# djene-mengistu/UAPS

Measured on AMD Instinct MI355X. Metric: training images/sec (labeled+unlabeled) NEU-Seg 256x256 K=3, higher is better.
Workload: dtype f32

## Files before the change

include/uaps_hip.h:

```cpp
#ifndef UAPS_HIP_H
#define UAPS_HIP_H

#include <stddef.h>
#include <stdint.h>

#ifdef __cplusplus
extern "C" {
#endif

typedef void* uaps_stream_t;

#define UAPS_MAX_HEADS 8
#define UAPS_MAX_CLASSES 8

#define UAPS_OK 0
#define UAPS_EINVAL (-1)
#define UAPS_ERANGE (-2)
#define UAPS_EWORKSPACE (-3)
#define UAPS_ENOFORM (-4)

int uaps_abi_version(void);
const char* uaps_error_string(int code);


// ... 426 lines not shown
#define UAPS_BIN_S_KBCE 15
#define UAPS_BIN_S_KFOCAL 16
#define UAPS_BIN_S_NSCALARS 24
int uaps_binloss_workspace_bytes(int B, int H, int W, size_t* out_host);
int uaps_binloss_fwd(const float* z, const void* target, const uaps_binloss_params* prm, int B, int H, int W, float* scalars,
                     void* workspace, size_t workspace_bytes, uaps_stream_t stream);
int uaps_binloss_bwd(const float* z, const void* target, const uaps_binloss_params* prm, const float* scalars, const float* grad,
                     int B, int H, int W, float* dz, uaps_stream_t stream);
int uaps_sigmoid_mse_fwd(const float* a, const float* b, long n, float* out, uaps_stream_t stream);
int uaps_sigmoid_mse_bwd(const float* a, const float* b, const float* g_map, long n, float* da, uaps_stream_t stream);
int uaps_sigmoid_kl_fwd(const float* a, const float* b, long n, float* out_mean, void* workspace, size_t workspace_bytes,
                        uaps_stream_t stream);
int uaps_sigmoid_kl_bwd(const float* a, const float* b, const float* grad, long n, float* da, uaps_stream_t stream);
int uaps_bin_confusion(const float* z, const int64_t* labels, int B, int H, int W, double threshold, int64_t* counts,
                       uaps_stream_t stream);

int uaps_add_relu(const float* a, const float* b, float* out, long n, uaps_stream_t stream);
int uaps_relu_bwd(const float* dout, const float* out, float* dx, long n, uaps_stream_t stream);
int uaps_bn_act_bwd_prepare(const float* dout, const float* y, const float* gamma, const float* beta, const float* save_mean,
                            const float* save_invstd, float slope, int B, int C, int H, int W, int groups, float* coef,
                            float* dgamma, float* dbeta, float* dconv_bias, float* dy_bound, void* workspace, size_t workspace_bytes,
                            uaps_stream_t stream);
int uaps_bn_act_bwd_finalize(const void* partials, int parts_per_image, const float* maxes, const float* gamma, const float* beta,
                             const float* save_mean, const float* save_invstd, int B, int C, int H, int W, int groups, float* coef,
                             float* dgamma, float* dbeta, float* dconv_bias, float* dy_bound, uaps_stream_t stream);
int uaps_bn_act_bwd_apply(const float* dout, const float* y, const float* coef, float slope, int B, int C, int H, int W, int groups,
                          float* dy, uaps_stream_t stream);
int uaps_head_bwd_fused(const float* dlogits, const float* y, const void* xf, float slope, int groups, const float* wb,
                        const float* dy_bound, float dy_mul, const float* x_bound, float x_mul, const float* save_mean,
                        const float* save_invstd, const float* gamma, const float* beta, int want_bias, int B, int Cin, int Cout,
                        int H, int W, int ks, int cfg, float* g, void* partials, float* maxes, void* workspace,
                        size_t workspace_bytes, uaps_stream_t stream);

int uaps_relu_bwd_sum(const float* const* dout_host, int k, const float* out, float* dx, long n, uaps_stream_t stream);

int uaps_cat2(const float* a, const float* b, float* out, long n, uaps_stream_t stream);

int uaps_augment_batch(const uint8_t* images_hwc, const uint8_t* masks, const int* params_i, const float* params_f,
                       const float* noise, uint64_t seed, int B, int Hs, int Ws, int Ho, int Wo, const float* mean3_host,
                       const float* std3_host, float* out, int64_t* out_mask, uaps_stream_t stream);

#define UAPS_AUG_END 0
#define UAPS_AUG_BC 1
#define UAPS_AUG_NOISE 2
#define UAPS_AUG_BLUR 3
#define UAPS_AUG_BRIGHT 4
#define UAPS_AUG_CONTRAST 5
#define UAPS_AUG_SATURATE 6
#define UAPS_AUG_HUE 7
#define UAPS_AUG_PIXDROP 8
#define UAPS_AUG_GRID 9
#define UAPS_AUG_MAX_OPS 8
typedef struct uaps_view_row {
    int32_t hflip, vflip, rot_k, grid_on;
    int32_t op[UAPS_AUG_MAX_OPS];
    float a[UAPS_AUG_MAX_OPS], b[UAPS_AUG_MAX_OPS];
} uaps_view_row;
typedef struct uaps_augment_views_call {
    uint32_t struct_size;
    int32_t V, B, Hs, Ws, Cs, Ho, Wo;
    const uint8_t* images;
    const uint8_t* masks;
    const uaps_view_row* rows_host;
    const uaps_view_row* rows;
    const float* grid_ys;
    const float* grid_xs;
// ... 281 lines not shown
```

uaps_amd/_lib.py:

```python
from __future__ import annotations

import ctypes as C
import os
import subprocess
import threading

from . import config

_HERE = os.path.dirname(os.path.abspath(__file__))
LIB_PATH = config.text("UAPS_HIP_LIB") or os.path.join(_HERE, "lib", "libuaps_hip.so")
CSRC = os.path.join(_HERE, "csrc")

_lock = threading.Lock()
_tls = threading.local()
_lib = None

c_float_p = C.POINTER(C.c_float)
c_void_p = C.c_void_p

_PTR = C.c_void_p
SIGNATURES = {
    "uaps_abi_version": (C.c_int, []),
    "uaps_error_string": (C.c_char_p, [C.c_int]),
    "uaps_loss_workspace_bytes": (C.c_int, [C.c_int] * 5 + [C.POINTER(C.c_size_t)]),
# ... 65 lines not shown
    "uaps_convs_fwd": (C.c_int, [_PTR] * 3 + [C.c_int] * 8 + [_PTR]),
    "uaps_convs_bwd_data": (C.c_int, [_PTR] * 3 + [C.c_int] * 8 + [_PTR]),
    "uaps_convs_wrw_workspace_bytes": (C.c_int, [C.c_int] * 8 + [C.POINTER(C.c_size_t)]),
    "uaps_convs_bwd_weight": (C.c_int, [_PTR] * 3 + [C.c_int] * 8 + [_PTR, C.c_size_t, _PTR]),
    "uaps_maxpool3x3s2_fwd": (C.c_int, [_PTR, _PTR, _PTR, C.c_long, C.c_int, C.c_int, _PTR]),
    "uaps_maxpool3x3s2_bwd": (C.c_int, [_PTR, _PTR, _PTR, C.c_long, C.c_int, C.c_int, _PTR]),
    "uaps_space_to_depth2": (C.c_int, [_PTR, _PTR, C.c_int, C.c_int, C.c_int, C.c_int, C.c_int, _PTR]),
    "uaps_subsample2_fwd": (C.c_int, [_PTR, _PTR, C.c_long, C.c_int, C.c_int, _PTR]),
    "uaps_subsample2_bwd": (C.c_int, [_PTR, _PTR, C.c_long, C.c_int, C.c_int, _PTR]),
    "uaps_sum_tensors": (C.c_int, [_PTR, C.c_int, _PTR, C.c_long, _PTR]),
    "uaps_pair_workspace_bytes": (C.c_int, [C.POINTER(C.c_size_t)]),
    "uaps_feat_dropout_stats": (C.c_int, [_PTR] + [C.c_int] * 4 + [_PTR, C.c_size_t, _PTR]),
    "uaps_fanout_perturbed": (C.c_int, [_PTR] * 7 + [C.c_int, C.c_int, C.c_uint64, C.c_float, C.c_float] + [C.c_int] * 4 + [_PTR]),
    "uaps_augment_batch": (C.c_int, [_PTR] * 5 + [C.c_uint64] + [C.c_int] * 5 + [C.POINTER(C.c_float), C.POINTER(C.c_float), _PTR, _PTR, _PTR]),
    "uaps_augment_views_workspace_bytes": (C.c_int, [C.c_int] * 4 + [C.POINTER(C.c_size_t)]),
    "uaps_augment_views": (C.c_int, [_PTR]),
    "uaps_softmax_klmap_bwd": (C.c_int, [_PTR] * 3 + [C.c_int] * 4 + [_PTR] * 3),
    "uaps_softmax_pair_fwd": (C.c_int, [_PTR, _PTR] + [C.c_int] * 5 + [_PTR, _PTR, _PTR, _PTR, C.c_size_t, _PTR]),
    "uaps_softmax_mse_bwd": (C.c_int, [_PTR] * 3 + [C.c_int] * 4 + [_PTR, _PTR]),
    "uaps_softmax_kl_bwd": (C.c_int, [_PTR] * 3 + [C.c_int] * 4 + [_PTR, _PTR]),
    "uaps_entropy_map": (C.c_int, [_PTR] + [C.c_int] * 4 + [_PTR, _PTR, _PTR, C.c_size_t, _PTR]),
    "uaps_fanin_perturbed": (C.c_int, [_PTR] * 4 + [C.c_int, C.c_int, C.c_uint64, C.c_float, C.c_float] + [C.c_int] * 4 + [_PTR, _PTR]),
    "uaps_maxpool2x2_fwd": (C.c_int, [_PTR] + [C.c_int] * 4 + [_PTR, _PTR, _PTR]),
    "uaps_adam_step": (C.c_int, [_PTR] * 5 + [C.c_int] + [C.c_double] * 5 + [C.c_long, _PTR]),
    "uaps_add_relu": (C.c_int, [_PTR, _PTR, _PTR, C.c_long, _PTR]),
    "uaps_relu_bwd": (C.c_int, [_PTR, _PTR, _PTR, C.c_long, _PTR]),
    "uaps_relu_bwd_sum": (C.c_int, [_PTR, C.c_int, _PTR, _PTR, C.c_long, _PTR]),
    "uaps_cat2": (C.c_int, [_PTR, _PTR, _PTR, C.c_long, _PTR]),
    "uaps_bn_act_bwd_prepare": (C.c_int, [_PTR] * 6 + [C.c_float] + [C.c_int] * 5 + [_PTR] * 6 + [C.c_size_t, _PTR]),
    "uaps_bn_act_bwd_apply": (C.c_int, [_PTR] * 3 + [C.c_float] + [C.c_int] * 5 + [_PTR, _PTR]),
    "uaps_bn_act_bwd_finalize": (C.c_int, [_PTR, C.c_int] + [_PTR] * 5 + [C.c_int] * 5 + [_PTR] * 6),
    "uaps_head_bwd_fused": (C.c_int, [_PTR] * 3 + [C.c_float, C.c_int, _PTR, _PTR, C.c_float, _PTR, C.c_float] + [_PTR] * 4 + [C.c_int] * 8 +
                            [_PTR] * 4 + [C.c_size_t, _PTR]),
    "uaps_seg_confusion": (C.c_int, [_PTR, _PTR] + [C.c_int] * 4 + [_PTR, _PTR]),
    "uaps_ema_update": (C.c_int, [_PTR] * 3 + [C.c_int, C.c_float, C.c_float, _PTR]),
    "uaps_teacher_noise": (C.c_int, [_PTR] + [C.c_int] * 5 + [C.c_uint64, C.c_uint64, _PTR, _PTR]),
    "uaps_teacher_noise_apply": (C.c_int, [_PTR, _PTR] + [C.c_int] * 5 + [_PTR, _PTR]),
    "uaps_mc_consistency_workspace_bytes": (C.c_int, [C.POINTER(C.c_size_t)]),
    "uaps_mc_consistency_fwd": (C.c_int, [_PTR] * 3 + [C.c_int] * 5 + [C.c_float] + [_PTR] * 4 + [C.c_size_t, _PTR]),
    "uaps_mc_consistency_bwd": (C.c_int, [_PTR] * 5 + [C.c_int] * 4 + [_PTR, _PTR]),
    "uaps_cct_dct_workspace_bytes": (C.c_int, [C.POINTER(C.c_size_t)]),
    "uaps_cct_consistency_fwd": (C.c_int, [_PTR] + [C.c_int] * 6 + [_PTR, _PTR, C.c_size_t, _PTR]),
    "uaps_cct_consistency_bwd": (C.c_int, [_PTR] + [C.c_int] * 6 + [_PTR, _PTR, _PTR]),
    "uaps_rot90_batch": (C.c_int, [_PTR, _PTR] + [C.c_int] * 5 + [_PTR, _PTR, _PTR]),
    "uaps_rot_consistency_fwd": (C.c_int, [_PTR, C.c_int, _PTR] + [C.c_int] * 6 + [_PTR, _PTR, C.c_size_t, _PTR]),
    "uaps_rot_consistency_bwd": (C.c_int, [_PTR, C.c_int, _PTR] + [C.c_int] * 6 + [_PTR, _PTR, _PTR, _PTR]),
    "uaps_cps_workspace_bytes": (C.c_int, [C.c_int] * 5 + [C.POINTER(C.c_size_t)]),
    "uaps_cps_fwd": (C.c_int, [_PTR] * 3 + [C.c_int] * 5 + [C.c_float] + [_PTR] * 4 + [C.c_size_t, _PTR]),
    "uaps_cps_bwd": (C.c_int, [_PTR] * 7 + [C.c_int] * 5 + [_PTR] * 3),
    "uaps_ucc_cutmix_batch": (C.c_int, [_PTR] * 6 + [C.c_int] * 4 + [_PTR] * 3),
    "uaps_ucc_workspace_bytes": (C.c_int, [C.c_int] * 4 + [C.POINTER(C.c_size_t)]),
    "uaps_ucc_fwd": (C.c_int, [_PTR] * 3 + [C.c_int] * 4 + [C.c_float] + [_PTR] * 6 + [C.c_size_t, _PTR]),
    "uaps_ucc_bwd": (C.c_int, [_PTR] * 6 + [C.c_int] * 4 + [_PTR] * 3),
    "uaps_segloss_workspace_bytes": (C.c_int, [C.c_int] * 4 + [C.POINTER(C.c_size_t)]),
    "uaps_segloss_fwd": (C.c_int, [_PTR] * 3 + [C.c_int] * 4 + [_PTR, _PTR, C.c_size_t, _PTR]),
    "uaps_segloss_bwd": (C.c_int, [_PTR] * 5 + [C.c_int] * 4 + [_PTR, _PTR]),
    "uaps_binloss_workspace_bytes": (C.c_int, [C.c_int] * 3 + [C.POINTER(C.c_size_t)]),
    "uaps_binloss_fwd": (C.c_int, [_PTR] * 3 + [C.c_int] * 3 + [_PTR, _PTR, C.c_size_t, _PTR]),
    "uaps_binloss_bwd": (C.c_int, [_PTR] * 5 + [C.c_int] * 3 + [_PTR, _PTR]),
    "uaps_sigmoid_mse_fwd": (C.c_int, [_PTR, _PTR, C.c_long, _PTR, _PTR]),
    "uaps_sigmoid_mse_bwd": (C.c_int, [_PTR, _PTR, _PTR, C.c_long, _PTR, _PTR]),
    "uaps_sigmoid_kl_fwd": (C.c_int, [_PTR, _PTR, C.c_long, _PTR, _PTR, C.c_size_t, _PTR]),
    "uaps_sigmoid_kl_bwd": (C.c_int, [_PTR, _PTR, _PTR, C.c_long, _PTR, _PTR]),
    "uaps_bin_confusion": (C.c_int, [_PTR, _PTR] + [C.c_int] * 3 + [C.c_double, _PTR, _PTR]),
    "uaps_tta_views": (C.c_int, [_PTR]),
    "uaps_tta_fold": (C.c_int, [_PTR]),
# ... 388 lines not shown
```

uaps_amd/config.py:

```python
from __future__ import annotations

import os
from typing import Dict

_seen: Dict[str, tuple] = {}

DOC = {
    "UAPS_HIP_LIB": "path of another build of libuaps_hip.so with the same ABI (same-box A/B of two kernel builds)",
    "UAPS_CONV_MODE": "arithmetic of the convolutions: 2 / h16 (default), 1 / split (exact three-piece bf16), 0 / exact (fp32 MFMA)",
    "UAPS_DEFER_WRW_REDUCE": "weight-gradient reductions batched behind the backward (conv.deferred_reduces)",
    "UAPS_EARLY_WRW_REDUCE": "... and the decoders' share of them on a side stream beside the encoder's backward",
    "UAPS_EARLY_ADAM": "the decoders' Adam step behind their early reductions (world size 1)",
    "UAPS_FUSED_UP2": "bilinear x2 formed in the staging of up4's first convolution instead of materialised",
    "UAPS_FUSED_BN_SUMS": "BatchNorm-backward sums in the epilogue of the 16 -> 16 input-gradient row kernel (measured a wash: off)",
    "UAPS_FUSED_HEAD_BWD": "out_conv's input gradient, weight gradient and the BatchNorm-backward sums behind it as one row pass (csrc/head_bwd_row.hip)",
    "UAPS_LAZY_BN_BWD": "BatchNorm backward in two halves on the 256-wide decoder layers (lazybn)",
    "UAPS_PAIR_CFG": "cfg bits of the pair-loss kernels (diagnosis)",
    "UAPS_FUSED_FANOUT": "all perturbed copies of a feature map written by one pass over it",
    "UAPS_EPILOGUE_STATS": "BatchNorm statistics in the producing convolution's epilogue",
    "UAPS_VIRTUAL_CAT": "two-source convolutions instead of a materialised torch.cat in the UpBlocks",
    "UAPS_FUSED_FAN": "perturbation backward fused into the gradient fan-in kernel",
    "UAPS_DECODER_CHAINS": "decoders are dealt round-robin onto this many streams (diagnosis)",
    "UAPS_FAN_BESIDE": "perturbed feature copies written on a side stream beside the encoder's next levels",
    "UAPS_PACK_BESIDE": "the decoders' weights packed on a side stream beside the encoder's forward",
    "UAPS_FUSED_POOL": "2x2 max-pool fused into the fan-out / fan-in kernels",
    "UAPS_FUSED_BN_CONV": "BatchNorm + LeakyReLU applied in the consuming convolution's staging",
    "UAPS_DECODER_STREAMS": "one HIP stream per auxiliary decoder (bench.py switches it on for the headline)",
    "UAPS_STAT_SHIFT": "BatchNorm partial sums formed about running_mean - conv bias",
    "UAPS_INPUT_IN_GRAPH": "the captured step reads the batch from its own static input buffers (filled by the concatenation kernel)",
}


def _raw(name: str):
    return os.environ.get(name)


def flag(name: str, default: bool) -> bool:
    v = _raw(name)
    val = default if v is None or v == "" else (v != "0")
    _seen[name] = (default, val)
    return val


def integer(name: str, default: int) -> int:
    v = _raw(name)
    val = default if v is None or v == "" else int(v)
    _seen[name] = (default, val)
    return val
# ... 16 lines not shown
```

uaps_amd/conv.py:

```python
from __future__ import annotations

import collections
import contextlib
import ctypes as C
import os
import weakref
from typing import Dict, Optional, Tuple

import torch
from torch.optim.optimizer import register_optimizer_step_post_hook

from . import _graddest, lazybn, _lib, bounds, config, stepctx

_ws = _lib.Workspace(min_bytes=1 << 22)
_packed: Dict[int, tuple] = {}
_generation = 0
_shared_cell = [0]


def optimizer_stepped(optimizer, *_args, **_kwargs) -> None:
    cell = getattr(optimizer, "_uaps_cell", None)
    if cell is None:
        cell = optimizer._uaps_cell = [0]
    cell[0] += 1
# ... 468 lines not shown
    B, Cin, H, W = x.shape
    y = torch.empty((B, Cout, H, W), dtype=torch.float32, device=x.device)
    L = _lib.lib()
    bp = bias.data_ptr() if bias is not None else None
    cfg = plan_cfg(ks, cfg, True, x, y)
    stats = None
    if want_stats:
        cfg = stats_cfg(cfg, xb)
        ppi = stats_parts_per_image(B, Cin, Cout, H, W, ks, cfg)
        stats = torch.empty((Cout, B, ppi, 2), dtype=torch.float32, device=x.device)
    am = _claim_amax(x.device)
    for attempt in range(2):
        hh = None
        if xb is not None or (want_stats and stat_shift is not None) or am is not None:
            hh = _lib.mk_hints((xb,) if xb is not None else (), am, stat_shift if want_stats else None)
        with _lib.device_guard(x.device), _timed(FWD, B, Cin, Cout, H, W, ks, cfg, hh, x=x, y=y, stats=stats):
            if want_stats:
                rc = L.uaps_conv_fwd_stats_h(hh, x.data_ptr(), wf.data_ptr(), bp, y.data_ptr(), stats.data_ptr(), B, Cin, Cout, H, W, ks, cfg,
                                             _lib.current_stream(x.device))
            else:
                rc = L.uaps_conv_fwd_h(hh, x.data_ptr(), wf.data_ptr(), bp, y.data_ptr(), B, Cin, Cout, H, W, ks, cfg,
                                       _lib.current_stream(x.device))
        if rc != ENOFORM or am is None:
            break
        am = None
    _lib.check(rc, "uaps_conv_fwd")
    _set_out_amax(am)
    return (y, stats, ppi) if want_stats else y


_FUSED_BSUM = config.flag("UAPS_FUSED_BN_SUMS", False)


def conv_bwd_data_raw(dy: torch.Tensor, wb: torch.Tensor, Cin: int, ks: int, cfg: int = 0, dyb=None, bsum=None, head=None):
    if head is not None and bsum is not None and head_bwd_eligible(dy, bsum[0], ks):
        res = head_bwd_fused(dy, dyb, bsum[0], head[0], head[1], wb, bsum[1], bsum[2], bsum[3], bsum[4], bsum[5], bsum[6], head[2], cfg, head[3])
        if res is not None:
            return res + (True,)
    B, Cout, H, W = dy.shape
    dev = dy.device
    dx = torch.empty((B, Cin, H, W), dtype=torch.float32, device=dev)
    cfg = plan_cfg(ks, cfg, True, dy, dx)
    L = _lib.lib()
    partials = maxes = None
    if bsum is not None and _FUSED_BSUM and dyb is not None and ks == 3 and Cin == 16 and Cout == 16 and W == 256 and H % 16 == 0:
        ppi = H // 16
        partials = torch.empty((Cin, B, ppi, 2), dtype=torch.float32, device=dev)
        maxes = torch.empty(2 * bounds.FLOATS, dtype=torch.float32, device=dev)
        with _lib.device_guard(dev):
            _lib.check(L.uaps_zero_bounds(maxes.data_ptr(), maxes.numel(), _lib.current_stream(dev)), "uaps_zero_bounds")
            hh = _lib.mk_hints((dyb,), bsum=(bsum[0], bsum[1], bsum[2], bsum[3], bsum[4], partials, maxes, bsum[5], bsum[6]))
            with _timed(BWD_DATA, B, Cin, Cout, H, W, ks, cfg, hh, x=dy, y=dx):
                rc = L.uaps_conv_bwd_data_h(hh, dy.data_ptr(), wb.data_ptr(), dx.data_ptr(), B, Cin, Cout, H, W, ks, cfg, _lib.current_stream(dev))
        if rc != ENOFORM:
            _lib.check(rc, "uaps_conv_bwd_data")
            return (dx, partials, maxes) + ((False,) if head is not None else ())
        partials = maxes = None
    hh = _lib.mk_hints((dyb,)) if dyb is not None else None
    with _lib.device_guard(dev), _timed(BWD_DATA, B, Cin, Cout, H, W, ks, cfg, hh, x=dy, y=dx):
        rc = L.uaps_conv_bwd_data_h(hh, dy.data_ptr(), wb.data_ptr(), dx.data_ptr(), B, Cin, Cout, H, W, ks, cfg, _lib.current_stream(dev))
    _lib.check(rc, "uaps_conv_bwd_data")
    if head is not None:
        return dx, None, None, False
    return (dx, None, None) if bsum is not None else dx


_FUSED_HEAD = config.flag("UAPS_FUSED_HEAD_BWD", True)
HEAD_BWD_KERNEL = "head_bwd_row_kernel"


def head_bwd_eligible(dz: torch.Tensor, y: torch.Tensor, ks: int) -> bool:
    return (_FUSED_HEAD and ks == 3 and y.shape[1] == 16 and dz.shape[1] <= 4 and y.shape[3] == 256 and y.shape[2] % 16 == 0
            and get_mode() == "h16")


def head_bwd_fused(dz: torch.Tensor, dzb, y: torch.Tensor, xf: torch.Tensor, xb, wb: torch.Tensor, mean, invstd, gamma, beta,
                   slope: float, groups: int, want_bias: bool, cfg: int, ws: torch.Tensor):
    B, Cout, H, W = dz.shape
    Cin = y.shape[1]
    dev = y.device
    g = torch.empty_like(y)
    partials = torch.empty((Cin, B, max(H // 16, 1), 2), dtype=torch.float32, device=dev)
    maxes = torch.empty(2 * bounds.FLOATS, dtype=torch.float32, device=dev)
    L = _lib.lib()
    on = KERNEL_EVENTS is not None and (EVENT_FILTER is None or HEAD_BWD_KERNEL in EVENT_FILTER)
    with _lib.device_guard(dev):
        st = _lib.current_stream(dev)
        _lib.check(L.uaps_zero_bounds(maxes.data_ptr(), maxes.numel(), st), "uaps_zero_bounds")
        with (_lib.LaunchTimer() if on else contextlib.nullcontext()) as timer:
            rc = L.uaps_head_bwd_fused(dz.data_ptr(), y.data_ptr(), xf.data_ptr(), float(slope), int(groups), wb.data_ptr(),
                                       dzb[0].data_ptr() if dzb is not None else None, float(dzb[1]) if dzb is not None else 1.0,
                                       xb[0].data_ptr() if xb is not None else None, float(xb[1]) if xb is not None else 1.0,
                                       mean.data_ptr(), invstd.data_ptr(), gamma.data_ptr(), beta.data_ptr(), int(want_bias), B, Cin, Cout,
                                       H, W, 3, cfg, g.data_ptr(), partials.data_ptr(), maxes.data_ptr(), ws.data_ptr(), ws.numel(), st)
        if on and rc == 0:
            KERNEL_EVENTS.setdefault(HEAD_BWD_KERNEL, []).append((timer.start, timer.stop, 2 * 2.0 * B * H * W * Cin * Cout * 9))
    if rc == ENOFORM:
        return None
    _lib.check(rc, "uaps_head_bwd_fused")
    return g, partials, maxes


def conv_bwd_weight_raw(dy: torch.Tensor, x: torch.Tensor, ks: int, want_bias: bool, cfg: int = 0, wkey=None, bkey=None,
                        dyb=None, xb=None, lz=None, prefs=None, step=None):
    B, Cout, H, W = dy.shape
    Cin = x.shape[1]
    dev = dy.device
    L = _lib.lib()
    n = C.c_size_t()
    cfg = plan_cfg(ks, cfg, True, dy, x)
    _lib.check(L.uaps_conv_wrw_workspace_bytes(B, Cin, Cout, H, W, ks, cfg, C.byref(n)), "uaps_conv_wrw_workspace_bytes")
    ws = _wrw_workspace(dev, n.value, prefs, step)
    dw = _graddest.take(wkey, (Cout, Cin, ks, ks), dev)
    db = _graddest.take(bkey, (Cout,), dev) if want_bias else None
    dy_true = None
    with _lib.device_guard(dev):
        st = _lib.current_stream(dev)
        rc = lazybn.ENOFORM
        if lz is not None and xb is not None:
            dy_true = torch.empty_like(dy)
            hh = _lib.mk_hints((lz.bound, xb), dyt=(lz.y, lz.coef, dy_true, lz.slope, lz.groups))
            with _timed(WRW, B, Cin, Cout, H, W, ks, cfg, hh, y_grad=dy, x=x):
                rc = L.uaps_conv_bwd_weight_partial_h(hh, dy.data_ptr(), x.data_ptr(), int(want_bias), B, Cin, Cout, H, W, ks, cfg,
                                                      ws.data_ptr(), ws.numel(), st)
            if rc != lazybn.ENOFORM:
                bounds.put(dy_true, *lz.bound)
        if lz is not None and rc == lazybn.ENOFORM:
            dy_true = dy = lazybn.materialize(dy, lz)
            dyb = bounds.get(dy)
        if lz is None or rc == lazybn.ENOFORM:
            hh = _lib.mk_hints((dyb, xb)) if (dyb is not None and xb is not None) else None
            with _timed(WRW, B, Cin, Cout, H, W, ks, cfg, hh, y_grad=dy, x=x):
# ... 402 lines not shown
```

uaps_amd/fused.py:

```python
from __future__ import annotations

import ctypes as C
from typing import Optional

import torch
import torch.nn as nn

from . import _graddest, lazybn, _lib, bounds, stepctx
from . import perturb as _perturb

_ws = _lib.Workspace(min_bytes=1 << 20)

def _groups() -> int:
    return stepctx.fwd().stat_groups


class stat_groups:

    def __init__(self, n: int):
        self.n = int(n)

    def __enter__(self):
        f = stepctx.fwd()
        self.prev, f.stat_groups = f.stat_groups, self.n
# ... 263 lines not shown
        slope, groups, has_cbias, has_bias, Cout, ks, cfg = ctx.meta
        lz_in = lazybn.take(dz)
        dzb, xb = bounds.get(dz), ctx.xb
        dz = dz.contiguous()
        B, Cc, H, W = y.shape
        dev = y.device
        L = _lib.lib()
        n = C.c_size_t()
        _lib.check(L.uaps_conv_wrw_workspace_bytes(B, Cc, Cout, H, W, ks, cfg, C.byref(n)), "uaps_conv_wrw_workspace_bytes")
        cws = _conv._wrw_workspace(dev, n.value, ctx.prefs, ctx.step)
        dw = _graddest.take(ctx.keys[3], (Cout, Cc, ks, ks), dev)
        want_db = has_bias and ctx.needs_input_grad[13]
        db = _graddest.take(ctx.keys[4], (Cout,), dev) if want_db else None

        def weight_gradient(dz, dzb, lz):
            out = torch.empty_like(dz) if lz is not None else None
            with _lib.device_guard(dev):
                st = _lib.current_stream(dev)
                hh = None
                if lz is not None:
                    hh = _lib.mk_hints((dzb, xb), dyt=(lz.y, lz.coef, out, lz.slope, lz.groups))
                elif dzb is not None and xb is not None:
                    hh = _lib.mk_hints((dzb, xb))
                with _conv._timed(_conv.WRW, B, Cc, Cout, H, W, ks, cfg, hh, y_grad=dz, x=y, xf=xf, xf_slope=slope, xf_groups=groups):
                    rc = L.uaps_conv_bwd_weight_partial_bn_h(hh, dz.data_ptr(), y.data_ptr(), xf.data_ptr(), slope, groups, int(want_db), B, Cc,
                                                           Cout, H, W, ks, cfg, cws.data_ptr(), cws.numel(), st)
                if lz is not None and rc == lazybn.ENOFORM:
                    return None
                _lib.check(rc, "uaps_conv_bwd_weight_partial_bn")
                _conv._wrw_reduce(cws, dw, db, B, Cc, Cout, H, W, ks, cfg, st, ctx.prefs, ctx.step)
            return bounds.put(out, *lz.bound) if lz is not None else dz

        done_w = False
        if lz_in is not None:
            out = weight_gradient(dz, lz_in.bound, lz_in) if xb is not None else None
            done_w = out is not None
            dz = out if done_w else lazybn.materialize(dz, lz_in)
            dzb = bounds.get(dz)
        lazy_up = ctx.lazy_up and not lazybn.observed(y)
        partials = maxes = None
        if lazy_up:
            head = (xf, xb, want_db, cws) if (not done_w and ctx.needs_input_grad[12]) else None
            res = _conv.conv_bwd_data_raw(dz, wb, Cc, ks, cfg, dyb=dzb, bsum=(y, stats[0], stats[1], gamma, beta, slope, groups), head=head)
            da, partials, maxes = res[:3]
            if head is not None and res[3]:
                with _lib.device_guard(dev):
                    _conv._wrw_reduce(cws, dw, db, B, Cc, Cout, H, W, ks, cfg, _lib.current_stream(dev), ctx.prefs, ctx.step)
                done_w = True
        else:
            da = _conv.conv_bwd_data_raw(dz, wb, Cc, ks, cfg, dyb=dzb)
        if not done_w:
            weight_gradient(dz, dzb, None)
        dgb = [_graddest.take(k, (Cc,), dev) for k in ctx.keys[:3]]
        ws = _bn_ws(dev, B, Cc, H, W)
        if lazy_up:
            if partials is not None:
                lazybn.prepare_from_partials(da, y, gamma, beta, stats[0], stats[1], slope, groups, dgb[0], dgb[1], dgb[2], partials, maxes, scope=ctx.lazy_scope)
            else:
                lazybn.prepare(da, y, gamma, beta, stats[0], stats[1], slope, groups, dgb[0], dgb[1], dgb[2], ws, scope=ctx.lazy_scope)
            dy = da
        else:
            dy = torch.empty_like(y)
            with _lib.device_guard(dev):
                st = _lib.current_stream(dev)
                am = bounds.new_amax(dev) if bounds.enabled() else None
                rc = L.uaps_bn_act_bwd_grouped_bias_h(_lib.mk_hints((), am) if am is not None else None, da.data_ptr(), y.data_ptr(), gamma.data_ptr(), beta.data_ptr(), stats[0].data_ptr(),
                                                    stats[1].data_ptr(), slope, 0.0, 0, 0, B, Cc, H, W, groups, dy.data_ptr(),
                                                    dgb[0].data_ptr(), dgb[1].data_ptr(), dgb[2].data_ptr(), ws.data_ptr(), ws.numel(), st)
                _lib.check(rc, "uaps_bn_act_bwd_grouped_bias")
            bounds.put(dy, am)
        return dy, None, (dgb[2] if has_cbias else None), dgb[0], dgb[1], None, None, None, None, None, None, None, dw, db, None, None, None


def can_fuse_bn_into_conv(y: torch.Tensor, weight: torch.Tensor) -> bool:
# ... 130 lines not shown
```

Before: 2638.

## Fuse 16->16 ConvBlock backward (wgrad, dgrad, BN sums) into one row kernel

New measurement: 2677, median of 6. 1.01x the previous value.

```diff
diff --git a/include/uaps_hip.h b/include/uaps_hip.h
--- a/include/uaps_hip.h
+++ b/include/uaps_hip.h
@@ -482,6 +482,12 @@
                         int H, int W, int ks, int cfg, float* g, void* partials, float* maxes, void* workspace,
                         size_t workspace_bytes, uaps_stream_t stream);
 
+int uaps_mid_bwd_fused(const float* dact, const float* y2, const float* coef, float slope2, int groups2, const float* y1,
+                       const void* xf, float slope, int groups, const float* wb, const float* dy_bound, float dy_mul,
+                       const float* x_bound, float x_mul, const float* save_mean, const float* save_invstd, const float* gamma,
+                       const float* beta, int want_bias, int B, int Cin, int Cout, int H, int W, int ks, int cfg, float* g,
+                       void* partials, float* maxes, void* workspace, size_t workspace_bytes, uaps_stream_t stream);
+
 int uaps_relu_bwd_sum(const float* const* dout_host, int k, const float* out, float* dx, long n, uaps_stream_t stream);
 
 int uaps_cat2(const float* a, const float* b, float* out, long n, uaps_stream_t stream);
diff --git a/uaps_amd/_lib.py b/uaps_amd/_lib.py
--- a/uaps_amd/_lib.py
+++ b/uaps_amd/_lib.py
@@ -121,6 +121,8 @@
     "uaps_bn_act_bwd_finalize": (C.c_int, [_PTR, C.c_int] + [_PTR] * 5 + [C.c_int] * 5 + [_PTR] * 6),
     "uaps_head_bwd_fused": (C.c_int, [_PTR] * 3 + [C.c_float, C.c_int, _PTR, _PTR, C.c_float, _PTR, C.c_float] + [_PTR] * 4 + [C.c_int] * 8 +
                             [_PTR] * 4 + [C.c_size_t, _PTR]),
+    "uaps_mid_bwd_fused": (C.c_int, [_PTR] * 3 + [C.c_float, C.c_int, _PTR, _PTR, C.c_float, C.c_int, _PTR, _PTR, C.c_float, _PTR, C.c_float] +
+                           [_PTR] * 4 + [C.c_int] * 8 + [_PTR] * 4 + [C.c_size_t, _PTR]),
     "uaps_seg_confusion": (C.c_int, [_PTR, _PTR] + [C.c_int] * 4 + [_PTR, _PTR]),
     "uaps_ema_update": (C.c_int, [_PTR] * 3 + [C.c_int, C.c_float, C.c_float, _PTR]),
     "uaps_teacher_noise": (C.c_int, [_PTR] + [C.c_int] * 5 + [C.c_uint64, C.c_uint64, _PTR, _PTR]),
diff --git a/uaps_amd/config.py b/uaps_amd/config.py
--- a/uaps_amd/config.py
+++ b/uaps_amd/config.py
@@ -14,6 +14,7 @@
     "UAPS_FUSED_UP2": "bilinear x2 formed in the staging of up4's first convolution instead of materialised",
     "UAPS_FUSED_BN_SUMS": "BatchNorm-backward sums in the epilogue of the 16 -> 16 input-gradient row kernel (measured a wash: off)",
     "UAPS_FUSED_HEAD_BWD": "out_conv's input gradient, weight gradient and the BatchNorm-backward sums behind it as one row pass (csrc/head_bwd_row.hip)",
+    "UAPS_FUSED_MID_BWD": "the 16 -> 16 convolution of a 256-wide ConvBlock: weight gradient, input gradient and the BatchNorm-backward sums behind it as one row pass (csrc/mid_bwd_row.hip)",
     "UAPS_LAZY_BN_BWD": "BatchNorm backward in two halves on the 256-wide decoder layers (lazybn)",
     "UAPS_PAIR_CFG": "cfg bits of the pair-loss kernels (diagnosis)",
     "UAPS_FUSED_FANOUT": "all perturbed copies of a feature map written by one pass over it",
diff --git a/uaps_amd/conv.py b/uaps_amd/conv.py
--- a/uaps_amd/conv.py
+++ b/uaps_amd/conv.py
@@ -524,7 +524,11 @@
 _FUSED_BSUM = config.flag("UAPS_FUSED_BN_SUMS", False)
 
 
-def conv_bwd_data_raw(dy: torch.Tensor, wb: torch.Tensor, Cin: int, ks: int, cfg: int = 0, dyb=None, bsum=None, head=None):
+def conv_bwd_data_raw(dy: torch.Tensor, wb: torch.Tensor, Cin: int, ks: int, cfg: int = 0, dyb=None, bsum=None, head=None, mid=None):
+    if mid is not None:
+        res = mid_bwd_fused(dy, mid[0], bsum[0], mid[1], mid[2], wb, bsum[1], bsum[2], bsum[3], bsum[4], bsum[5], bsum[6], mid[3], cfg, mid[4]) \
+            if bsum is not None and mid_bwd_eligible(dy, bsum[0], ks) else None
+        return res + (True,) if res is not None else (None, None, None, False)
     if head is not None and bsum is not None and head_bwd_eligible(dy, bsum[0], ks):
         res = head_bwd_fused(dy, dyb, bsum[0], head[0], head[1], wb, bsum[1], bsum[2], bsum[3], bsum[4], bsum[5], bsum[6], head[2], cfg, head[3])
         if res is not None:
@@ -590,6 +594,45 @@
     if rc == ENOFORM:
         return None
     _lib.check(rc, "uaps_head_bwd_fused")
+    return g, partials, maxes
+
+
+_FUSED_MID = config.flag("UAPS_FUSED_MID_BWD", True)
+MID_BWD_KERNEL = "mid_bwd_row_kernel"
+
+
+def mid_bwd_eligible(dz: torch.Tensor, y: torch.Tensor, ks: int) -> bool:
+    return (_FUSED_MID and ks == 3 and y.shape[1] == 16 and dz.shape[1] == 16 and y.shape[3] == 256 and y.shape[2] % 16 == 0
+            and get_mode() == "h16")
+
+
+def mid_bwd_fused(dz: torch.Tensor, lz, y: torch.Tensor, xf: torch.Tensor, xb, wb: torch.Tensor, mean, invstd, gamma, beta,
+                  slope: float, groups: int, want_bias: bool, cfg: int, ws: torch.Tensor):
+    B, Cout, H, W = dz.shape
+    Cin = y.shape[1]
+    dev = y.device
+    g = torch.empty_like(y)
+    partials = torch.empty((Cin, B, max(H // 16, 1), 2), dtype=torch.float32, device=dev)
+    maxes = torch.empty(2 * bounds.FLOATS, dtype=torch.float32, device=dev)
+    dzb = lz.bound if lz is not None else None
+    L = _lib.lib()
+    on = KERNEL_EVENTS is not None and (EVENT_FILTER is None or MID_BWD_KERNEL in EVENT_FILTER)
+    with _lib.device_guard(dev):
+        st = _lib.current_stream(dev)
+        _lib.check(L.uaps_zero_bounds(maxes.data_ptr(), maxes.numel(), st), "uaps_zero_bounds")
+        with (_lib.LaunchTimer() if on else contextlib.nullcontext()) as timer:
+            rc = L.uaps_mid_bwd_fused(dz.data_ptr(), lz.y.data_ptr() if lz is not None else None, lz.coef.data_ptr() if lz is not None else None,
+                                      float(lz.slope) if lz is not None else 0.0, int(lz.groups) if lz is not None else 1,
+                                      y.data_ptr(), xf.data_ptr(), float(slope), int(groups), wb.data_ptr(),
+                                      dzb[0].data_ptr() if dzb is not None else None, float(dzb[1]) if dzb is not None else 1.0,
+                                      xb[0].data_ptr() if xb is not None else None, float(xb[1]) if xb is not None else 1.0,
+                                      mean.data_ptr(), invstd.data_ptr(), gamma.data_ptr(), beta.data_ptr(), int(want_bias), B, Cin, Cout,
+                                      H, W, 3, cfg, g.data_ptr(), partials.data_ptr(), maxes.data_ptr(), ws.data_ptr(), ws.numel(), st)
+        if on and rc == 0:
+            KERNEL_EVENTS.setdefault(MID_BWD_KERNEL, []).append((timer.start, timer.stop, 2 * 2.0 * B * H * W * Cin * Cout * 9))
+    if rc == ENOFORM:
+        return None
+    _lib.check(rc, "uaps_mid_bwd_fused")
     return g, partials, maxes
 
 
diff --git a/uaps_amd/csrc/mid_bwd_row.hip b/uaps_amd/csrc/mid_bwd_row.hip
--- /dev/null
+++ b/uaps_amd/csrc/mid_bwd_row.hip
@@ -0,0 +1,462 @@
+#include "../../include/uaps_hip.h"
+#include "conv_kernels.hpp"
+#include "conv_split.hpp"
+#include "hints.hpp"
+
+extern "C" int uaps_conv_get_mode(void);
+extern "C" unsigned uaps_conv_get_tuning(void);
+
+namespace uaps {
+
+struct MidBwdArgs {
+    const float* dact;
+    const float* y2;
+    const float* coef;
+    float dt_slope;
+    int dt_Bg;
+    const float* y1;
+    const float2* xf;
+    float slope;
+    int Bg;
+    const float* wp;
+    const float* wscale;
+    int CGP;
+    float* g;
+    float* slab; float* bslab; int nsplit;
+    const float* dy_bound; const float* in_bound;
+    float dy_mul, in_mul;
+    const float* bs_mean; const float* bs_invstd; const float* bs_gamma; const float* bs_beta;
+    float2* partials;
+    float* bs_max;
+    unsigned* err;
+    int B, H;
+};
+
+__global__ __launch_bounds__(512, 2) void mid_bwd_row_kernel(MidBwdArgs a) {
+    constexpr int WIDTH = 256, NG = WIDTH / 8, XG = NG + 2, NSLOT = 3, ROWS = 16, CI = 16, NTHR = 512, NXL = 4;
+    constexpr int X_UNITS = 2 * CI * NSLOT * XG;
+    constexpr int D_UNITS = 2 * 16 * NG;
+    constexpr int IW = WIDTH + 8, CGU = NSLOT * IW, PIECE = 2 * CGU, XS = 3;
+    constexpr int NQ = 9 * 2, NSTEP = (NQ + 3) / 4, MW = 4;
+    constexpr int GS = WIDTH + 4;
+    constexpr int RED_FLOATS = 2 * 10 * 256;
+    static_assert(RED_FLOATS / 4 <= X_UNITS, "the reduction scratch fits the input image");
+
+    __shared__ __attribute__((aligned(16))) u32x4 sX[X_UNITS];
+    __shared__ __attribute__((aligned(16))) u32x4 sD[2 * D_UNITS];
+    __shared__ __attribute__((aligned(16))) u32x4 sIn[2 * PIECE];
+    __shared__ __attribute__((aligned(16))) float sG[16 * GS];
+
+    const f32x2 sd = h16_scale(__builtin_fmaxf(bound_of(a.dy_bound, a.dy_mul), 0.f));
+    const f32x2 sx = h16_scale(__builtin_fmaxf(bound_of(a.in_bound, a.in_mul), 0.f));
+    const float sc_d = sd.x, inv_d = sd.y, sc_x = sx.x, inv_x = sx.y;
+
+    const int tid = threadIdx.x, lane = tid & 63, wave = tid >> 6;
+    const int j = lane & 15, kq = lane >> 4;
+    const int wave_u = __builtin_amdgcn_readfirstlane(wave);
+    const int W = WIDTH, HW = a.H * W;
+    const uint32_t HW4 = (uint32_t)HW * 4u;
+
+    const int split = xcd_swizzle(blockIdx.x, gridDim.x);
+    if (split >= a.nsplit) return;
+    const int rpi = a.H / ROWS, nruns = a.B * rpi;
+    const int run_begin = (int)((long)nruns * split / a.nsplit), run_end = (int)((long)nruns * (split + 1) / a.nsplit);
+
+    for (int e = tid; e < 2 * CI * NSLOT * 2; e += NTHR) sX[(e / 2) * XG + (e % 2) * (XG - 1)] = u32x4{0u, 0u, 0u, 0u};
+    for (int e = tid; e < 2 * 2 * NSLOT * 8; e += NTHR) sIn[(e / 8) * IW + (e % 8 < 4 ? e % 8 : IW - 8 + e % 8)] = u32x4{0u, 0u, 0u, 0u};
+
+    float bs_md = 0.f, bs_mx = 0.f;
+
+    if (wave_u < 4) {
+        const int sp = wave_u;
+        const int dc0 = wave_u * 4, cg = wave_u >> 1, ch = wave_u & 1;
+        const bool want_bias = a.bslab != nullptr;
+        f32x4 rd[4], ry[4];
+        bool d_in = false;
+        float dtc[4][6];
+        auto ld4 = [](__amdgpu_buffer_rsrc_t rs, uint32_t off) { return __builtin_bit_cast(f32x4, __builtin_amdgcn_raw_buffer_load_b128(rs, (int)off, 0, 0)); };
+        auto load_d = [&](int b, int gy, f32x4 (&dd)[4], f32x4 (&yy)[4], bool& ok) {
+            ok = (unsigned)gy < (unsigned)a.H;
+            const __amdgpu_buffer_rsrc_t rsd = make_rsrc(a.dact + (size_t)b * 16 * HW, 16u * HW4);
+            const __amdgpu_buffer_rsrc_t rsy = make_rsrc(a.y2 + (size_t)b * 16 * HW, 16u * HW4);
+            const uint32_t off = (uint32_t)(dc0 * HW + gy * W + lane * 4) * 4u;
+#pragma unroll
+            for (int i = 0; i < 4; ++i) dd[i] = ld4(rsd, ok ? off + (uint32_t)i * HW4 : kOob);
+#pragma unroll
+            for (int i = 0; i < 4; ++i) yy[i] = ld4(rsy, ok ? off + (uint32_t)i * HW4 : kOob);
+        };
+        auto store_d = [&](f32x4 (&dd)[4], f32x4 (&yy)[4], bool ok, int slot, int buf) {
+            float v[4][4];
+#pragma unroll
+            for (int i = 0; i < 4; ++i) {
+                asm volatile("" : "+v"(dd[i]));
+                asm volatile("" : "+v"(yy[i]));
+#pragma unroll
+                for (int k = 0; k < 4; ++k) {
+                    const float g0 = dd[i][k];
+                    const float yc = yy[i][k] - dtc[i][0];
+                    const float z = yc * dtc[i][2] + dtc[i][3];
+                    const float d = z > 0.f ? g0 : g0 * a.dt_slope;
+                    const float t = dtc[i][2] * (d - dtc[i][4] - (yc * dtc[i][1]) * dtc[i][5]);
+                    v[i][k] = ok ? t : 0.f;
+                }
+            }
+            const int base = (cg * NSLOT + slot) * IW + 4 + lane * 4;
+#pragma unroll
+            for (int k = 0; k < 4; ++k) {
+                unsigned q00, q01, q10, q11;
+                conv_split2h(v[0][k] * sc_d, v[1][k] * sc_d, q00, q01);
+                conv_split2h(v[2][k] * sc_d, v[3][k] * sc_d, q10, q11);
+                *reinterpret_cast<uint2*>(reinterpret_cast<unsigned*>(&sIn[base + k]) + ch * 2) = make_uint2(q00, q10);
+                *reinterpret_cast<uint2*>(reinterpret_cast<unsigned*>(&sIn[PIECE + base + k]) + ch * 2) = make_uint2(q01, q11);
+            }
+            if (buf >= 0) {
+#pragma unroll
+                for (int i = 0; i < 4; ++i) {
+                    unsigned a0, a1, b0, b1;
+                    conv_split2h(v[i][0] * sc_d, v[i][1] * sc_d, a0, a1);
+                    conv_split2h(v[i][2] * sc_d, v[i][3] * sc_d, b0, b1);
+                    const int c = dc0 + i;
+                    *reinterpret_cast<uint2*>(reinterpret_cast<unsigned*>(&sD[buf * D_UNITS + c * NG]) + lane * 2) = make_uint2(a0, b0);
+                    *reinterpret_cast<uint2*>(reinterpret_cast<unsigned*>(&sD[buf * D_UNITS + (16 + c) * NG]) + lane * 2) = make_uint2(a1, b1);
+                }
+            }
+        };
+
+        f32x4 acc[9];
+        f32x4 accb = f32x4{0.f, 0.f, 0.f, 0.f};
+#pragma unroll
+        for (int t = 0; t < 9; ++t) acc[t] = f32x4{0.f, 0.f, 0.f, 0.f};
+        constexpr unsigned kOnes = 0x3C003C00u;
+        const f16x8 ones = __builtin_bit_cast(f16x8, u32x4{kOnes, kOnes, kOnes, kOnes});
+
+        for (int run = run_begin; run < run_end; ++run) {
+            const int b = run / rpi, r0 = (run % rpi) * ROWS;
+            const int grp2 = b / a.dt_Bg;
+#pragma unroll
+            for (int i = 0; i < 4; ++i)
+#pragma unroll
+                for (int k = 0; k < 6; ++k) dtc[i][k] = a.coef[((size_t)grp2 * 16 + dc0 + i) * 8 + k];
+            {
+                f32x4 da[4], ya[4], db[4], yb[4];
+                bool oka, okb;
+                load_d(b, r0 - 1, da, ya, oka);
+                load_d(b, r0, db, yb, okb);
+                load_d(b, r0 + 1, rd, ry, d_in);
+                __builtin_amdgcn_sched_barrier(0);
+                store_d(da, ya, oka, 0, -1);
+                store_d(db, yb, okb, 1, 0);
+                store_d(rd, ry, d_in, 2, 1);
+            }
+            __syncthreads();
+            int s0 = 0, buf = 0;
+#pragma unroll 1
+            for (int t = r0; t < r0 + ROWS; ++t) {
+                const bool more = t + 1 < r0 + ROWS;
+                if (more) load_d(b, t + 2, rd, ry, d_in);
+                const int s1 = s0 + 1 >= NSLOT ? s0 + 1 - NSLOT : s0 + 1, s2 = s1 + 1 >= NSLOT ? s1 + 1 - NSLOT : s1 + 1;
+                const u32x4* sDb = sD + buf * D_UNITS;
+#pragma unroll
+                for (int sgi = 0; sgi < 2; ++sgi) {
+                    const int gq = (sp * 2 + sgi) * 4 + kq;
+                    f16x8 af[2];
+#pragma unroll
+                    for (int p = 0; p < 2; ++p) af[p] = __builtin_bit_cast(f16x8, sDb[(p * 16 + j) * NG + gq]);
+                    if (want_bias) {
+                        accb = __builtin_amdgcn_mfma_f32_16x16x32_f16(af[1], ones, accb, 0, 0, 0);
+                        accb = __builtin_amdgcn_mfma_f32_16x16x32_f16(af[0], ones, accb, 0, 0, 0);
+                    }
+#pragma unroll
+                    for (int ky = 0; ky < 3; ++ky) {
+                        const int slot = ky == 0 ? s0 : (ky == 1 ? s1 : s2);
+                        f16x8 bf[3][2];
+#pragma unroll
+                        for (int p = 0; p < 2; ++p) {
+                            const int u = ((p * CI + j) * NSLOT + slot) * XG + gq + 1;
+                            const u32x4 c = sX[u];
+                            const unsigned cl3 = reinterpret_cast<const unsigned*>(&sX[u - 1])[3];
+                            const unsigned cr0 = reinterpret_cast<const unsigned*>(&sX[u + 1])[0];
+                            const unsigned t01 = __builtin_amdgcn_alignbit(c[1], c[0], 16), t12 = __builtin_amdgcn_alignbit(c[2], c[1], 16);
+                            const unsigned t23 = __builtin_amdgcn_alignbit(c[3], c[2], 16);
+                            const unsigned tE0 = __builtin_amdgcn_alignbit(c[0], cl3, 16), t3E = __builtin_amdgcn_alignbit(cr0, c[3], 16);
+                            bf[0][p] = __builtin_bit_cast(f16x8, u32x4{tE0, t01, t12, t23});
+                            bf[1][p] = __builtin_bit_cast(f16x8, c);
+                            bf[2][p] = __builtin_bit_cast(f16x8, u32x4{t01, t12, t23, t3E});
+                        }
+#pragma unroll
+                        for (int kx = 0; kx < 3; ++kx) {
+                            f32x4 c = acc[ky * 3 + kx];
+                            c = __builtin_amdgcn_mfma_f32_16x16x32_f16(af[1], bf[kx][0], c, 0, 0, 0);
+                            c = __builtin_amdgcn_mfma_f32_16x16x32_f16(af[0], bf[kx][1], c, 0, 0, 0);
+                            c = __builtin_amdgcn_mfma_f32_16x16x32_f16(af[0], bf[kx][0], c, 0, 0, 0);
+                            acc[ky * 3 + kx] = c;
+                        }
+                    }
+                }
+                __syncthreads();
+                if (more) store_d(rd, ry, d_in, s0, buf);
+                s0 = s1; buf ^= 1;
+                __syncthreads();
+            }
+        }
+
+        float* red = reinterpret_cast<float*>(sX);
+#pragma unroll
+        for (int s = 2; s >= 1; s >>= 1) {
+            if (sp >= s && sp < 2 * s) {
+                float* p = red + (size_t)(sp - s) * 10 * 256 + lane;
+#pragma unroll
+                for (int t = 0; t < 9; ++t)
+#pragma unroll
+                    for (int r = 0; r < 4; ++r) p[(t * 4 + r) * 64] = acc[t][r];
+#pragma unroll
+                for (int r = 0; r < 4; ++r) p[(36 + r) * 64] = accb[r];
+            }
+            __syncthreads();
+            if (sp < s) {
+                const float* p = red + (size_t)sp * 10 * 256 + lane;
+#pragma unroll
+                for (int t = 0; t < 9; ++t)
+#pragma unroll
+                    for (int r = 0; r < 4; ++r) acc[t][r] += p[(t * 4 + r) * 64];
+#pragma unroll
+                for (int r = 0; r < 4; ++r) accb[r] += p[(36 + r) * 64];
+            }
+            __syncthreads();
+        }
+        if (sp == 0) {
+            float* slab = a.slab + (size_t)split * 9 * 16 * CI;
+            float chk = 0.f;
+            const float inv = inv_d * inv_x;
+#pragma unroll
+            for (int t = 0; t < 9; ++t) {
+                note_nonfinite(chk, acc[t]);
+#pragma unroll
+                for (int r = 0; r < 4; ++r) slab[((size_t)t * 16 + kq * 4 + r) * CI + j] = acc[t][r] * inv;
+            }
+            report_nonfinite(a.err, chk, UAPS_ERR_WRW_NONFINITE);
+            if (want_bias && j == 0) {
+                float inv_b = inv_d;
+                asm volatile("" : "+v"(inv_b));
+#pragma unroll
+                for (int r = 0; r < 4; ++r) a.bslab[(size_t)split * 16 + kq * 4 + r] = accb[r] * inv_b;
+            }
+        }
+    } else {
+        const int wg = wave_u - 4;
+        const int xc0 = wg * NXL;
+        const float out_scale_a = inv_d, out_scale_w = a.wscale[1];
+
+        u32x4 bfr[NSTEP][2];
+        int kxo[NSTEP], kyv[NSTEP];
+        {
+            const __amdgpu_buffer_rsrc_t rs_w = make_rsrc(a.wp, (uint32_t)(2 * 9) * a.CGP * 16u * 16u);
+#pragma unroll
+            for (int s = 0; s < NSTEP; ++s) {
+                const int q = 4 * s + kq, tap = q / 2, cgq = q % 2;
+#pragma unroll
+                for (int p = 0; p < 2; ++p) {
+                    const uint32_t off = q < NQ ? (uint32_t)(((p * 9 + tap) * a.CGP + cgq) * 16 + j) * 16u : kOob;
+                    bfr[s][p] = __builtin_amdgcn_raw_buffer_load_b128(rs_w, (int)off, 0, 0);
+                }
+                const int qq = q < NQ ? q : 0;
+                kxo[s] = (qq % 2) * CGU + (qq / 2) % 3; kyv[s] = (qq / 2) / 3;
+            }
+        }
+        int abase[MW];
+#pragma unroll
+        for (int m = 0; m < MW; ++m) abase[m] = (wg * MW + m) * 16 + j + XS;
+
+        f32x4 rx[NXL], xa[NXL], xb[NXL];
+        f32x2 cf[NXL];
+        float bs_mu[NXL], bs_is[NXL], bs_sc[NXL], bs_sh[NXL];
+        bool x_in = false;
+        auto ld4 = [](__amdgpu_buffer_rsrc_t rs, uint32_t off) { return __builtin_bit_cast(f32x4, __builtin_amdgcn_raw_buffer_load_b128(rs, (int)off, 0, 0)); };
+        auto load_x = [&](int b, int gy, f32x4 (&dst)[NXL], bool& ok) {
+            ok = (unsigned)gy < (unsigned)a.H;
+            const __amdgpu_buffer_rsrc_t rs = make_rsrc(a.y1 + (size_t)b * CI * HW, (uint32_t)CI * HW4);
+            const uint32_t off = (uint32_t)(xc0 * HW + gy * W + lane * 4) * 4u;
+#pragma unroll
+            for (int i = 0; i < NXL; ++i) dst[i] = ld4(rs, ok ? off + (uint32_t)i * HW4 : kOob);
+        };
+        auto store_x = [&](f32x4 (&src)[NXL], bool ok, int slot) {
+#pragma unroll
+            for (int i = 0; i < NXL; ++i) {
+                asm volatile("" : "+v"(src[i]));
+                float v[4];
+#pragma unroll
+                for (int k = 0; k < 4; ++k) {
+                    const float z = __builtin_fmaf(src[i][k], cf[i].x, cf[i].y);
+                    v[k] = ok ? __builtin_fmaxf(z, z * a.slope) : 0.f;
+                }
+                unsigned a0, a1, b0, b1;
+                conv_split2h(v[0] * sc_x, v[1] * sc_x, a0, a1);
+                conv_split2h(v[2] * sc_x, v[3] * sc_x, b0, b1);
+                const int c = xc0 + i;
+                unsigned* p0 = reinterpret_cast<unsigned*>(&sX[(c * NSLOT + slot) * XG + 1]) + lane * 2;
+                unsigned* p1 = reinterpret_cast<unsigned*>(&sX[((CI + c) * NSLOT + slot) * XG + 1]) + lane * 2;
+                *reinterpret_cast<uint2*>(p0) = make_uint2(a0, b0);
+                *reinterpret_cast<uint2*>(p1) = make_uint2(a1, b1);
+            }
+        };
+
+        for (int run = run_begin; run < run_end; ++run) {
+            const int b = run / rpi, r0 = (run % rpi) * ROWS;
+            const int grp = b / a.Bg;
+            float st_s[NXL][4], st_q[NXL][4];
+#pragma unroll
+            for (int i = 0; i < NXL; ++i) {
+                const int c = xc0 + i;
+                const float2 t = a.xf[(size_t)grp * CI + c];
+                cf[i] = f32x2{t.x, t.y};
+                bs_mu[i] = a.bs_mean[grp * CI + c]; bs_is[i] = a.bs_invstd[grp * CI + c];
+                bs_sc[i] = a.bs_gamma[c] * bs_is[i]; bs_sh[i] = a.bs_beta[c];
+#pragma unroll
+                for (int v = 0; v < 4; ++v) { st_s[i][v] = 0.f; st_q[i][v] = 0.f; }
+            }
+            {
+                f32x4 ra[NXL];
+                bool oka, okb;
+                load_x(b, r0 - 1, ra, oka);
+                load_x(b, r0, xa, okb);
+                load_x(b, r0 + 1, xb, x_in);
+                __builtin_amdgcn_sched_barrier(0);
+                store_x(ra, oka, 0);
+                store_x(xa, okb, 1);
+                store_x(xb, x_in, 2);
+            }
+            __syncthreads();
+            int s0 = 0;
+            const __amdgpu_buffer_rsrc_t rs_g = make_rsrc(a.g + (size_t)b * CI * HW, (uint32_t)CI * HW4);
+#pragma unroll 1
+            for (int t = r0; t < r0 + ROWS; ++t) {
+                const bool more = t + 1 < r0 + ROWS;
+                if (more) load_x(b, t + 2, rx, x_in);
+                const int s1 = s0 + 1 >= NSLOT ? s0 + 1 - NSLOT : s0 + 1, s2 = s1 + 1 >= NSLOT ? s1 + 1 - NSLOT : s1 + 1;
+
+                int aoff[NSTEP];
+#pragma unroll
+                for (int s = 0; s < NSTEP; ++s) aoff[s] = kxo[s] + (kyv[s] == 0 ? s0 : (kyv[s] == 1 ? s1 : s2)) * IW;
+                f32x4 gacc[MW];
+#pragma unroll
+                for (int m = 0; m < MW; ++m) gacc[m] = f32x4{0.f, 0.f, 0.f, 0.f};
+                constexpr int NUN = NSTEP * MW;
+                u32x4 af[2][2];
+                auto read_a = [&](int u, u32x4 (&dst)[2]) {
+                    const int s = u / MW, m = u % MW;
+#pragma unroll
+                    for (int p = 0; p < 2; ++p) dst[p] = sIn[p * PIECE + abase[m] + aoff[s]];
+                };
+                read_a(0, af[0]);
+#pragma unroll
+                for (int u = 0; u < NUN; ++u) {
+                    const int s = u / MW, m = u % MW;
+                    if (u + 1 < NUN) read_a(u + 1, af[(u + 1) & 1]);
+                    const auto Hf = [](const u32x4& v) { return __builtin_bit_cast(f16x8, v); };
+                    f32x4 c = gacc[m];
+                    c = __builtin_amdgcn_mfma_f32_16x16x32_f16(Hf(af[u & 1][1]), Hf(bfr[s][0]), c, 0, 0, 0);
+                    c = __builtin_amdgcn_mfma_f32_16x16x32_f16(Hf(af[u & 1][0]), Hf(bfr[s][1]), c, 0, 0, 0);
+                    c = __builtin_amdgcn_mfma_f32_16x16x32_f16(Hf(af[u & 1][0]), Hf(bfr[s][0]), c, 0, 0, 0);
+                    gacc[m] = c;
+                    if (u + 1 < NUN) __builtin_amdgcn_sched_group_barrier(0x100, 2, 0);
+                    __builtin_amdgcn_sched_group_barrier(0x008, 3, 0);
+                }
+                float chk = 0.f;
+#pragma unroll
+                for (int m = 0; m < MW; ++m) {
+                    f32x4 v = gacc[m];
+                    v *= out_scale_a; v *= out_scale_w;
+                    v += 0.f;
+                    note_nonfinite(chk, v);
+                    *reinterpret_cast<f32x4*>(&sG[j * GS + (wg * MW + m) * 16 + kq * 4]) = v;
+                }
+                report_nonfinite(a.err, chk, UAPS_ERR_CONV_NONFINITE);
+                __syncthreads();
+
+#pragma unroll
+                for (int i = 0; i < NXL; ++i) {
+                    const f32x4 gv = *reinterpret_cast<const f32x4*>(&sG[(xc0 + i) * GS + lane * 4]);
+                    __builtin_amdgcn_raw_buffer_store_b128(__builtin_bit_cast(u32x4, gv), rs_g, (int)((uint32_t)((xc0 + i) * HW + t * W + lane * 4) * 4u), 0, 0);
+                    float cs = st_s[i][0], cq = st_q[i][0];
+#pragma unroll
+                    for (int e = 0; e < 4; ++e) {
+                        const float yc = xa[i][e] - bs_mu[i], z = yc * bs_sc[i] + bs_sh[i];
+                        const float d = z > 0.f ? gv[e] : gv[e] * a.slope, xh = yc * bs_is[i];
+                        cs += d; cq += d * xh;
+                        bs_md = __builtin_fmaxf(bs_md, __builtin_fabsf(d)); bs_mx = __builtin_fmaxf(bs_mx, __builtin_fabsf(xh));
+                    }
+#pragma unroll
+                    for (int v = 0; v < 3; ++v) { st_s[i][v] = st_s[i][v + 1]; st_q[i][v] = st_q[i][v + 1]; }
+                    st_s[i][3] = cs; st_q[i][3] = cq;
+                }
+                if (more) store_x(rx, x_in, s0);
+#pragma unroll
+                for (int i = 0; i < NXL; ++i) { xa[i] = xb[i]; xb[i] = rx[i]; }
+                s0 = s1;
+                __syncthreads();
+            }
+#pragma unroll
+            for (int i = 0; i < NXL; ++i) {
+                float s = 0.f, q = 0.f;
+#pragma unroll
+                for (int v = 0; v < 4; ++v) {
+                    float sv = st_s[i][v], qv = st_q[i][v];
+#pragma unroll
+                    for (int o = 32; o > 0; o >>= 1) { sv += __shfl_xor(sv, o, 64); qv += __shfl_xor(qv, o, 64); }
+                    s = v == 0 ? sv : s + sv; q = v == 0 ? qv : q + qv;
+                }
+                if (lane == 0) a.partials[((size_t)(xc0 + i) * a.B + b) * rpi + r0 / ROWS] = make_float2(s, q);
+            }
+        }
+        __syncthreads(); __syncthreads(); __syncthreads(); __syncthreads();
+    }
+    block_amax_to(a.bs_max, bs_md, sG);
+    block_amax_to(a.bs_max + UAPS_BOUND_FLOATS, bs_mx, sG + 16);
+}
+
+}
+
+extern "C" int uaps_mid_bwd_fused(const float* dact, const float* y2, const float* coef, float slope2, int groups2, const float* y1,
+                                  const void* xf, float slope, int groups, const float* wb, const float* dy_bound, float dy_mul,
+                                  const float* x_bound, float x_mul, const float* save_mean, const float* save_invstd,
+                                  const float* gamma, const float* beta, int want_bias, int B, int Cin, int Cout, int H, int W, int ks,
+                                  int cfg, float* g, void* partials, float* maxes, void* ws, size_t ws_bytes, uaps_stream_t stream) {
+    if (!dact || !y1 || !xf || !wb || !save_mean || !save_invstd || !gamma || !beta || !g || !partials || !maxes || !ws) return UAPS_EINVAL;
+    if (B <= 0 || Cin <= 0 || Cout <= 0 || H <= 0 || W <= 0 || groups < 1 || B % groups || (uintptr_t)xf % 8) return UAPS_EINVAL;
+    if ((y2 || coef) && (!y2 || !coef || groups2 < 1 || B % groups2)) return UAPS_EINVAL;
+    if (!(slope >= 0.f && slope <= 1.f)) return UAPS_ERANGE;
+    if (ks != 3 || Cin != 16 || Cout != 16 || W != 256 || H % 16 || H > 65536 || (cfg & ~0x3ff)) return UAPS_ENOFORM;
+    if (!y2 || !coef) return UAPS_ENOFORM;
+    if (uaps_conv_get_mode() != 2 || !dy_bound || !x_bound) return UAPS_ENOFORM;
+    if (uaps_conv_get_tuning() & (UAPS_TUNE_NO_ROW_WRW | UAPS_TUNE_NO_SPLIT_WRW)) return UAPS_ENOFORM;
+    if (((uintptr_t)dact | (uintptr_t)y2 | (uintptr_t)y1 | (uintptr_t)g | (uintptr_t)wb | (uintptr_t)ws | (uintptr_t)coef) % 16) return UAPS_ENOFORM;
+    size_t need = 0;
+    const int rc = uaps_conv_wrw_workspace_bytes(B, Cin, Cout, H, W, ks, cfg, &need);
+    if (rc) return rc;
+    constexpr int CoutS = 16, CinS = 16;
+    const size_t per_split = ((size_t)9 * CoutS * CinS + CoutS) * sizeof(float);
+    if (need == 0 || need % per_split) return UAPS_ENOFORM;
+    const int nsplit = (int)(need / per_split);
+    if (ws_bytes < need) return UAPS_EWORKSPACE;
+    uaps::account_bytes(4.0 * B * H * W * (3.0 * Cout + 1.0 * Cin));
+    uaps::MidBwdArgs a{};
+    a.dact = dact; a.y2 = y2; a.coef = coef; a.dt_slope = slope2; a.dt_Bg = B / groups2;
+    a.y1 = y1; a.xf = (const float2*)xf; a.slope = slope; a.Bg = B / groups;
+    const int CGP = uaps::split_cgroups(Cout);
+    const float* split_w = wb + (size_t)9 * ((Cout + 7) / 8 * 8) * ((Cin + 15) / 16 * 16);
+    const size_t piece = (size_t)9 * CGP * ((Cin + 15) / 16 * 16) * 4;
+    a.wscale = split_w + 3 * piece + 16;
+    a.wp = split_w + 3 * piece + uaps::kH16Header;
+    a.CGP = CGP;
+    a.g = g;
+    a.slab = (float*)ws; a.nsplit = nsplit;
+    a.bslab = want_bias ? a.slab + (size_t)nsplit * 9 * CoutS * CinS : nullptr;
+    a.dy_bound = dy_bound; a.dy_mul = dy_mul; a.in_bound = x_bound; a.in_mul = x_mul;
+    a.bs_mean = save_mean; a.bs_invstd = save_invstd; a.bs_gamma = gamma; a.bs_beta = beta;
+    a.partials = (float2*)partials; a.bs_max = maxes;
+    a.err = uaps::error_word();
+    a.B = B; a.H = H;
+    const unsigned grid = (unsigned)((nsplit + 7) / 8 * 8);
+    UAPS_LAUNCH_MAIN(uaps::mid_bwd_row_kernel, dim3(grid), dim3(512), 0, (hipStream_t)stream, a);
+    return (int)hipGetLastError();
+}
diff --git a/uaps_amd/fused.py b/uaps_amd/fused.py
--- a/uaps_amd/fused.py
+++ b/uaps_amd/fused.py
@@ -319,14 +319,24 @@
             return bounds.put(out, *lz.bound) if lz is not None else dz
 
         done_w = False
-        if lz_in is not None:
+        lazy_up = ctx.lazy_up and not lazybn.observed(y)
+        da = partials = maxes = None
+        if lz_in is not None and lazy_up and xb is not None and ctx.needs_input_grad[12] and _conv.mid_bwd_eligible(dz, y, ks):
+            res = _conv.conv_bwd_data_raw(dz, wb, Cc, ks, cfg, dyb=lz_in.bound, bsum=(y, stats[0], stats[1], gamma, beta, slope, groups),
+                                          mid=(lz_in, xf, xb, want_db, cws))
+            if res[3]:
+                da, partials, maxes = res[:3]
+                with _lib.device_guard(dev):
+                    _conv._wrw_reduce(cws, dw, db, B, Cc, Cout, H, W, ks, cfg, _lib.current_stream(dev), ctx.prefs, ctx.step)
+                done_w = True
+        if lz_in is not None and da is None:
             out = weight_gradient(dz, lz_in.bound, lz_in) if xb is not None else None
             done_w = out is not None
             dz = out if done_w else lazybn.materialize(dz, lz_in)
             dzb = bounds.get(dz)
-        lazy_up = ctx.lazy_up and not lazybn.observed(y)
-        partials = maxes = None
-        if lazy_up:
+        if da is not None:
+            pass
+        elif lazy_up:
             head = (xf, xb, want_db, cws) if (not done_w and ctx.needs_input_grad[12]) else None
             res = _conv.conv_bwd_data_raw(dz, wb, Cc, ks, cfg, dyb=dzb, bsum=(y, stats[0], stats[1], gamma, beta, slope, groups), head=head)
             da, partials, maxes = res[:3]
```
